# ext-sakamoro/ALICE-Codec

Hardware: AMD Instinct MI355X
Metric: Mpixels/s encode+decode, 1080p x 64 CDF9/7 q=80; bit-exact vs CPU (higher is better)
Workload: dtype int32

## Files before the change

alice-codec_amd/csrc/rans.hip:

```cpp
#include <cstdlib>

#include "common.h"
#include "freq_table.h"
#include "kernels.h"

namespace alice {


__device__ inline RansEncEntry make_enc_entry(uint32_t f, uint32_t c) {
    RansEncEntry e;
    e.freq = f;
    e.cum = c;
    unsigned long long xm = (unsigned long long)f << 19;
    unsigned long long xm8 = (unsigned long long)f << 27;
    e.xmax = xm > 0xFFFFFFFFull ? 0xFFFFFFFFu : (uint32_t)xm;
    e.xmax8 = xm8 > 0xFFFFFFFFull ? 0xFFFFFFFFu : (uint32_t)xm8;
    if (f == 0u || f > kProbScale) {
        e.xmax = f == 0u ? 0xFFFFFFFFu : e.xmax;
        e.xmax8 = f == 0u ? 0xFFFFFFFFu : e.xmax8;
        e.rcp = 0u; e.rsh = 0u; e.g = 0; e.cbias = 0u;
    } else if (f == 1u) {
        e.rcp = 0xFFFFFFFFu; e.rsh = 0u; e.g = 4095; e.cbias = c + 4095u;
    } else {
        uint32_t L = 32u - (uint32_t)__clz((int)(f - 1u));
        unsigned long long p = 1ull << (31u + L);
        e.rcp = (uint32_t)((p + f - 1u) / f);
        e.rsh = L - 1u;
        e.g = (int32_t)kProbScale - (int32_t)f;
        e.cbias = c;
    }
    return e;
}

__device__ inline uint32_t build_dec_slots(uint32_t f, uint32_t c, uint32_t* scratch, RansDecSlots* __restrict__ out) {
    const int s = threadIdx.x;
    uint32_t end = c + f;
    if (end > kProbScale) end = kProbScale;
    __syncthreads();
    scratch[s] = c;
    scratch[256 + s] = c < end ? end : c;
    scratch[512 + s] = f;
    out->symtab[s] = (f & 0xFFFFu) | (c << 16);
    __syncthreads();
    uint32_t fl = 0u;
    for (uint32_t slot = (uint32_t)s; slot < kProbScale; slot += 256u) {
        uint32_t owner = 0u;
        for (uint32_t k = 0; k < 256u; ++k)
            if (slot >= scratch[k] && slot < scratch[256 + k]) owner = k;
        const uint32_t fo = scratch[512 + owner], co = scratch[owner];
        uint32_t fe, be;
        if (fo >= kProbScale) {
            fe = 0xFFFFFFFFu; be = (slot - co) - slot + 1u;
            fl |= fo > kProbScale ? kTableDecExact : kTableDecBig;
        } else {
            fe = fo << 20; be = (slot - co) - ((fo * slot) >> kProbBits);
        }
        out->ftab[slot] = fe;
        out->btab[slot] = be;
        out->c2s[slot] = (uint8_t)owner;
    }
    return fl;
}

__global__ __launch_bounds__(256) void rans_table_kernel(const uint32_t* __restrict__ hist,
                                                         RansTable* __restrict__ tables, uint32_t n_sym,
                                                         const uint32_t* __restrict__ used) {
    __shared__ uint32_t scratch[768];
    const int chain = blockIdx.x;
    const int s = threadIdx.x;
    const uint32_t count = (uint32_t)s < n_sym ? hist[(size_t)chain * 256 + s] : 0u;
    uint32_t f, c;
    freq_table_256(count, n_sym, scratch, f, c);
    tables[chain].enc[s] = make_enc_entry(f, c);
    uint32_t fl = build_dec_slots(f, c, scratch, &tables[chain].dec);
    const uint32_t occurs = used ? used[(size_t)chain * 256 + s] : count;
    if (occurs > 0u && f == 0u) fl |= kTableDiverges;
    if (occurs > 0u && f > kProbScale) fl |= kTableNeedsGeneric;
    __shared__ uint32_t flags_sh;
    if (s == 0) flags_sh = 0u;
    __syncthreads();
    if (fl) atomicOr(&flags_sh, fl);
    __syncthreads();
    if (s == 0) tables[chain].flags = flags_sh | kTableVerified;
}

__global__ __launch_bounds__(256) void rans_table_from_arrays_kernel(const uint16_t* __restrict__ cum,
                                                                     const uint16_t* __restrict__ freq,
                                                                     RansTable* __restrict__ table) {
    __shared__ uint32_t scratch[768];
    __shared__ uint32_t flags_sh;
    const int s = threadIdx.x;
    if (s == 0) flags_sh = 0u;
    table->enc[s] = make_enc_entry(freq[s], cum[s]);
    const uint32_t fl = build_dec_slots(freq[s], cum[s], scratch, &table->dec);
    if (fl) atomicOr(&flags_sh, fl);
    __syncthreads();
    if (s == 0) table->flags = flags_sh;
}

__device__ __forceinline__ void chain_take_turns(uint32_t enabled) {
    if (!enabled) return;
    const uint32_t turn = (uint32_t)(clock64() >> 17);
    const uint32_t slot = __builtin_amdgcn_s_getreg((3 << 11) | (0 << 6) | 4);
    if ((turn ^ slot) & 1u) __builtin_amdgcn_s_setprio(1);
    else __builtin_amdgcn_s_setprio(0);
}


constexpr int kEncTile = 1024;
constexpr int kEncTilePad = 128;

__device__ __forceinline__ void ripple64(uint32_t& xin, uint32_t& xout, uint32_t xmax, uint32_t xmax8,
                                         uint32_t rcp, uint32_t rsh, int32_t g, uint32_t cprev) {
    uint32_t k, y, q;
    unsigned long long m1;
#define ALICE_RIPPLE_STEP(TAIL)                                                     \
    "v_add_u32_dpp %[xin], %[xout], %[cprev] wave_shr:1 row_mask:0xf bank_mask:0xf\n\t" \
    "v_cmp_ge_u32_e64 %[m1], %[xin], %[xmax]\n\t"                                  \
    "v_cmp_ge_u32_e32 vcc, %[xin], %[xmax8]\n\t"                                   \
    "s_nop 0\n\t"                                                                    \
    "v_cndmask_b32_e64 %[k], 0, 8, %[m1]\n\t"                                      \
    "v_cndmask_b32_e64 %[k], %[k], 16, vcc\n\t"                                    \
    "v_lshrrev_b32_e32 %[y], %[k], %[xin]\n\t"                                     \
    "v_mul_hi_u32 %[q], %[y], %[rcp]\n\t"                                          \
    "v_lshrrev_b32_e32 %[q], %[rsh], %[q]\n\t"                                     \
    "v_mad_i32_i24 %[xout], %[q], %[g], %[y]\n\t" TAIL
#define ALICE_RIPPLE_STEP4 ALICE_RIPPLE_STEP("s_nop 1\n\t") ALICE_RIPPLE_STEP("s_nop 1\n\t") ALICE_RIPPLE_STEP("s_nop 1\n\t") ALICE_RIPPLE_STEP("s_nop 1\n\t")
#define ALICE_RIPPLE_STEP16 ALICE_RIPPLE_STEP4 ALICE_RIPPLE_STEP4 ALICE_RIPPLE_STEP4 ALICE_RIPPLE_STEP4
    asm volatile(
        "s_nop 1\n\t"
        ALICE_RIPPLE_STEP16 ALICE_RIPPLE_STEP16 ALICE_RIPPLE_STEP16 ALICE_RIPPLE_STEP16
        : [xin] "+v"(xin), [xout] "+v"(xout), [k] "=&v"(k), [y] "=&v"(y), [q] "=&v"(q), [m1] "=&s"(m1)
        : [xmax] "v"(xmax), [xmax8] "v"(xmax8), [rcp] "v"(rcp), [rsh] "v"(rsh), [g] "v"(g),
          [cprev] "v"(cprev)
        : "vcc");
#undef ALICE_RIPPLE_STEP16
#undef ALICE_RIPPLE_STEP4
#undef ALICE_RIPPLE_STEP
}

__device__ __forceinline__ void ripple64_clean(uint32_t& xin, uint32_t& xout, uint32_t thr, uint32_t k0, uint32_t k1,
                                               uint32_t rcp, uint32_t rsh, int32_t g, uint32_t cprev) {
    uint32_t k, y, q;
#define ALICE_RIPPLE_STEP                                                            \
    "v_add_u32_dpp %[xin], %[xout], %[cprev] wave_shr:1 row_mask:0xf bank_mask:0xf\n\t" \
    "v_cmp_ge_u32_e32 vcc, %[xin], %[thr]\n\t"                                     \
    "s_nop 1\n\t"                                                                  \
    "v_cndmask_b32_e32 %[k], %[k0], %[k1], vcc\n\t"                                \
    "v_lshrrev_b32_e32 %[y], %[k], %[xin]\n\t"                                     \
    "v_mul_hi_u32 %[q], %[y], %[rcp]\n\t"                                          \
    "v_lshrrev_b32_e32 %[q], %[rsh], %[q]\n\t"                                     \
    "v_mad_i32_i24 %[xout], %[q], %[g], %[y]\n\t"                                  \
    "s_nop 1\n\t"
#define ALICE_RIPPLE_STEP4 ALICE_RIPPLE_STEP ALICE_RIPPLE_STEP ALICE_RIPPLE_STEP ALICE_RIPPLE_STEP
#define ALICE_RIPPLE_STEP16 ALICE_RIPPLE_STEP4 ALICE_RIPPLE_STEP4 ALICE_RIPPLE_STEP4 ALICE_RIPPLE_STEP4
    asm volatile(
        "s_nop 1\n\t"
        ALICE_RIPPLE_STEP16 ALICE_RIPPLE_STEP16 ALICE_RIPPLE_STEP16 ALICE_RIPPLE_STEP16
        : [xin] "+v"(xin), [xout] "+v"(xout), [k] "=&v"(k), [y] "=&v"(y), [q] "=&v"(q)
        : [thr] "v"(thr), [k0] "v"(k0), [k1] "v"(k1), [rcp] "v"(rcp), [rsh] "v"(rsh), [g] "v"(g), [cprev] "v"(cprev)
        : "vcc");
#undef ALICE_RIPPLE_STEP16
#undef ALICE_RIPPLE_STEP4
#undef ALICE_RIPPLE_STEP
}

__device__ __forceinline__ void ripple64_comp(uint32_t& u, uint32_t& z, uint32_t kc, uint32_t tpp, uint32_t rcp, uint32_t rsh,
                                              int32_t g) {
    uint32_t m, q;
#define ALICE_RIPPLE_STEP                                                            \
    "v_add_u32_dpp %[u], %[z], %[kc] wave_shr:1 row_mask:0xf bank_mask:0xf\n\t"     \
    "v_mad_i64_i32 v[62:63], vcc, %[u], %[two24], v[60:61]\n\t"                    \
    "v_min_u32_e32 %[m], %[u], v63\n\t"                                           \
    "v_mul_hi_u32 %[q], %[m], %[rcp]\n\t"                                          \
    "v_lshrrev_b32_e32 %[q], %[rsh], %[q]\n\t"                                     \
    "v_mad_i32_i24 %[z], %[q], %[g], %[m]\n\t"                                     \
    "s_nop 1\n\t"
#define ALICE_RIPPLE_STEP4 ALICE_RIPPLE_STEP ALICE_RIPPLE_STEP ALICE_RIPPLE_STEP ALICE_RIPPLE_STEP
#define ALICE_RIPPLE_STEP16 ALICE_RIPPLE_STEP4 ALICE_RIPPLE_STEP4 ALICE_RIPPLE_STEP4 ALICE_RIPPLE_STEP4
    asm volatile(
        "v_mov_b32_e32 v60, 0\n\t"
        "v_mov_b32_e32 v61, %[tpp]\n\t"
        ALICE_RIPPLE_STEP16 ALICE_RIPPLE_STEP16 ALICE_RIPPLE_STEP16 ALICE_RIPPLE_STEP16
        : [u] "+v"(u), [z] "=&v"(z), [m] "=&v"(m), [q] "=&v"(q)
        : [kc] "v"(kc), [tpp] "v"(tpp), [rcp] "v"(rcp), [rsh] "v"(rsh), [g] "v"(g), [two24] "s"(1u << 24)
        : "v60", "v61", "v62", "v63", "vcc");
#undef ALICE_RIPPLE_STEP16
#undef ALICE_RIPPLE_STEP4
#undef ALICE_RIPPLE_STEP
}

template <bool kExclusive>
__global__ __launch_bounds__(64) void rans_encode_kernel(const uint8_t* __restrict__ sym_base,
                                                         unsigned long long sym_stride,
                                                         unsigned long long n_first,
                                                         const RansTable* __restrict__ tables,
                                                         uint8_t* __restrict__ out_base,
                                                         unsigned long long cap0,
                                                         unsigned long long group_stride,
                                                         unsigned long long group_head,
                                                         unsigned n_split,
                                                         RansResult* __restrict__ results,
                                                         unsigned long long cap1, unsigned long long cap2,
                                                         uint32_t x_init, uint32_t keep_open, uint32_t take_turns,
                                                         const RansEncodeDesc* __restrict__ descs) {
    __shared__ uint4 tab_a[256];
    __shared__ uint4 tab_b[256];
    __shared__ uint2 tab_c[256];
    __shared__ __attribute__((aligned(16))) uint8_t tile[kEncTilePad + kEncTile];

    if constexpr (kExclusive) asm volatile("" ::: "a255");
    const int chain = blockIdx.x;
    const int lane = threadIdx.x;
    unsigned long long n = n_first - (((unsigned)chain >= n_split && n_first > 0ull) ? 1ull : 0ull);
    const uint8_t* __restrict__ sym = sym_base + (size_t)chain * sym_stride;
    const RansTable* __restrict__ tbl = tables + chain;
    const int gch = chain % 3;
    unsigned long long cap = group_stride == 0ull ? cap0 : (gch == 0 ? cap0 : (gch == 1 ? cap1 : cap2));
    uint8_t* region = group_stride == 0ull ? out_base + (size_t)chain * cap0
                                           : out_base + (size_t)(chain / 3) * group_stride + group_head +
                                                 (gch == 0 ? 0ull : (gch == 1 ? cap0 : cap0 + cap1));
    RansResult* res = results + chain;
    if (descs) {
        const RansEncodeDesc ds = descs[chain];
        sym = ds.sym; n = ds.n; tbl = ds.table; region = ds.region; cap = ds.cap; res = ds.result;
        x_init = ds.x_init; keep_open = ds.keep_open;
    }
    uint8_t* const out_end = region + cap;
    uint8_t* const dummy = region + lane;

    for (int s = lane; s < 256; s += 64) {
        const RansEncEntry e = tbl->enc[s];
        tab_a[s] = make_uint4(e.xmax, e.rcp, e.rsh, (uint32_t)e.g);
        tab_b[s] = make_uint4(e.xmax - (e.xmax >> 8), e.cbias + e.freq + ((1u << 31) - kProbScale - 1u), e.cbias, e.xmax8);
        tab_c[s] = make_uint2(e.freq, e.cum);
    }

    const uint32_t tbl_flags = (uint32_t)__builtin_amdgcn_readfirstlane((int)tbl->flags);
    const bool table_clean = x_init == kRansL && (tbl_flags & (kTableVerified | kTableNeedsGeneric | kTableDiverges)) == kTableVerified;
    uint32_t x = x_init;
    const unsigned long long clk0 = clock64(), rt0 = wall_clock64();
    unsigned long long written = 0ull;
    uint32_t flags = 0u;
    uint32_t paths = 0u, load_paths = 0u, slow_tiles = 0u, comp_blocks = 0u;
    asm volatile("" : "+v"(load_paths));

    const unsigned long long ntiles = (n + kEncTile - 1) / kEncTile;
    auto load_tile = [&](unsigned long long j) -> uint4 {
        uint4 v = make_uint4(0u, 0u, 0u, 0u);
        if (j >= ntiles) return v;
        const long long hi = (long long)(n - j * kEncTile);
        const long long lo = hi - kEncTile + 16ll * lane;
        if (lo >= 0) {
            const uint8_t* p = sym + lo;
            const uint32_t mis = (uint32_t)((uintptr_t)p & 3u);
            const uint32_t* p4 = (const uint32_t*)(p - mis);
            if (mis == 0u) {
                v = make_uint4(p4[0], p4[1], p4[2], p4[3]);
            } else if (lo + 20 <= (long long)n || mis == 0u) {
                const uint32_t t0 = p4[0], t1 = p4[1], t2 = p4[2], t3 = p4[3], t4 = p4[4];
                const uint32_t sh = mis * 8u;
                load_paths |= kEncPathFunnel;
                v = make_uint4((t0 >> sh) | (t1 << (32u - sh)), (t1 >> sh) | (t2 << (32u - sh)),
                               (t2 >> sh) | (t3 << (32u - sh)), (t3 >> sh) | (t4 << (32u - sh)));
            } else {
                uint32_t w[4] = {0u, 0u, 0u, 0u};
                for (int b = 0; b < 16; ++b) w[b >> 2] |= (uint32_t)p[b] << (8 * (b & 3));
                v = make_uint4(w[0], w[1], w[2], w[3]);
                load_paths |= kEncPathBytewiseEnd;
            }
        } else {
            uint32_t w[4] = {0u, 0u, 0u, 0u};
            for (int b = 0; b < 16; ++b) {
                const long long idx = lo + b;
                if (idx >= 0) w[b >> 2] |= (uint32_t)sym[idx] << (8 * (b & 3));
            }
            v = make_uint4(w[0], w[1], w[2], w[3]);
            load_paths |= kEncPathBytewiseHead;
        }
        return v;
    };

    struct BlockParams { uint4 ea, eb; uint2 ec; };
    auto sym_of = [&](int b) -> uint32_t { return tile[kEncTilePad + kEncTile - 1 - lane - b * 64]; };
    auto params_of = [&](uint32_t s) -> BlockParams { BlockParams p; p.ea = tab_a[s]; p.eb = tab_b[s]; p.ec = tab_c[s]; return p; };

    uint4 cur = load_tile(0);
    for (unsigned long long j = 0; j < ntiles; ++j) {
        if (!kExclusive && (j & 7ull) == 0ull) chain_take_turns(take_turns);
        __syncthreads();
        ((uint4*)(tile + kEncTilePad))[lane] = cur;
        __syncthreads();
        cur = load_tile(j + 1);
        const long long hi = (long long)(n - j * kEncTile);
        const int valid = hi >= kEncTile ? kEncTile : (int)hi;
        const int nblocks = (valid + 63) / 64;

        uint32_t sym1 = sym_of(1);
        BlockParams nxt = params_of(sym_of(0));
        if (table_clean && valid == kEncTile && written + 2ull * kEncTile + 4ull + 320ull <= cap) {
            uint32_t xin = x;
            constexpr uint32_t kTileSpan = 2u * kEncTile + 320u;
            const uintptr_t tb_v = (uintptr_t)(out_end - written - kTileSpan);
            typedef __attribute__((address_space(1))) uint8_t GlobalByte;
            GlobalByte* const tb = (GlobalByte*)(((uintptr_t)(uint32_t)__builtin_amdgcn_readfirstlane((int)(uint32_t)(tb_v >> 32)) << 32) |
                                                 (uintptr_t)(uint32_t)__builtin_amdgcn_readfirstlane((int)(uint32_t)tb_v));
            uint32_t tw = 0u, rare_blocks = 0u;
            asm volatile("" : "+v"(tw));
#pragma unroll 2
            for (int b = 0; b < kEncTile / 64; ++b) {
                const BlockParams curp = nxt;
                nxt = params_of(sym1);
                sym1 = sym_of(b + 2);
                const uint32_t xmax = curp.ea.x, rcp = curp.ea.y, rsh = curp.ea.z;
                const int32_t g = (int32_t)curp.ea.w;
                const bool small_f = xmax <= kRansL;
                if (__builtin_expect(__ballot(small_f) == 0ull, 1)) {
                    const uint32_t tm1 = xmax - 1u, tpp = curp.eb.x, cc = curp.eb.y;
                    uint32_t cc_prev = (uint32_t)__builtin_amdgcn_update_dpp(0, (int)cc, 0x138, 0xf, 0xf, true);
                    asm volatile("" : "+v"(cc_prev));
                    const uint32_t kc = tm1 - cc_prev;
                    uint32_t u = tm1 - xin, z;
                    ripple64_comp(u, z, kc, tpp, rcp, rsh, g);
                    const bool c1 = (int32_t)u < 0;
                    const unsigned long long b1 = __ballot(c1);
                    const uint32_t off = __builtin_amdgcn_mbcnt_hi((uint32_t)(b1 >> 32), __builtin_amdgcn_mbcnt_lo((uint32_t)b1, tw));
                    tb[c1 ? kTileSpan - 1u - off : (uint32_t)lane] = (uint8_t)(~u & 0xFFu);
                    tw += (uint32_t)__popcll(b1);
                    xin = (uint32_t)__builtin_amdgcn_update_dpp(0, (int)(cc - z), 0x13C, 0xf, 0xf, true);
                } else {
                    rare_blocks += 1u;
                    const uint32_t cbias = curp.eb.z, xmax8 = curp.eb.w;
                    uint32_t xout = 0u;
                    const uint32_t cprev = (uint32_t)__builtin_amdgcn_update_dpp(0, (int)cbias, 0x138, 0xf, 0xf, true);
                    const uint32_t k0 = small_f ? 8u : 0u;
                    ripple64_clean(xin, xout, small_f ? xmax8 : xmax, k0, k0 + 8u, rcp, rsh, g, cprev);
                    const bool c1 = xin >= xmax;
                    const bool c2 = xin >= xmax8;
                    const unsigned long long b1 = __ballot(c1), b2 = __ballot(c2);
                    const uint32_t off = __builtin_amdgcn_mbcnt_hi((uint32_t)(b1 >> 32), __builtin_amdgcn_mbcnt_lo((uint32_t)b1, tw)) +
                                         __builtin_amdgcn_mbcnt_hi((uint32_t)(b2 >> 32), __builtin_amdgcn_mbcnt_lo((uint32_t)b2, 0u));
                    tb[c1 ? kTileSpan - 1u - off : (uint32_t)lane] = (uint8_t)(xin & 0xFFu);
                    tb[c2 ? kTileSpan - 2u - off : (uint32_t)lane] = (uint8_t)((xin >> 8) & 0xFFu);
                    tw += (uint32_t)__popcll(b1) + (uint32_t)__popcll(b2);
                    xin = (uint32_t)__builtin_amdgcn_update_dpp(0, (int)(xout + cbias), 0x13C, 0xf, 0xf, false);
                }
                asm volatile("" : "+v"(tw));
            }
            written += (unsigned long long)(uint32_t)__builtin_amdgcn_readfirstlane((int)tw);
            comp_blocks += (uint32_t)(kEncTile / 64) - rare_blocks;
            x = (uint32_t)__builtin_amdgcn_readlane((int)xin, 0);
            continue;
        }
        slow_tiles += 1u;
        paths |= valid < kEncTile ? kEncPathTail : (table_clean ? kEncPathCapRefused : kEncPathNotClean);
        for (int b = 0; b < nblocks; ++b) {
            const BlockParams curp = nxt;
            nxt = params_of(sym1);
            sym1 = sym_of(b + 2);
            const bool active = (kEncTile - 1 - (b * 64 + lane)) >= kEncTile - valid;
            uint4 ea = curp.ea;
            uint4 eb = curp.eb;
            uint2 ec = curp.ec;
            if (!active) {
                ea = make_uint4(0xFFFFFFFFu, 0u, 0u, 0u);
                eb = make_uint4(0u, 0u, 0u, 0xFFFFFFFFu);
                ec = make_uint2(1u, 0u);
            }
            const uint32_t xmax = ea.x, xmax8 = eb.w, rcp = ea.y, rsh = ea.z;
            const int32_t g = (int32_t)ea.w;
            const uint32_t cbias = eb.z, freq = ec.x, cum = ec.y;
            const bool bad = (freq - 1u) >= kProbScale;

            uint32_t xin = x, xout = 0u;
            if (__builtin_expect(__ballot(bad) == 0ull, 1)) {
                uint32_t cprev = (uint32_t)__builtin_amdgcn_update_dpp(0, (int)cbias, 0x138, 0xf, 0xf, true);
                ripple64(xin, xout, xmax, xmax8, rcp, rsh, g, cprev);
                x = (uint32_t)__builtin_amdgcn_readlane((int)xout, 63) +
                    (uint32_t)__builtin_amdgcn_readlane((int)cbias, 63);
            } else {
                paths |= kEncPathExact;
                uint32_t xs = x;
                for (int i = 0; i < 64; ++i) {
                    if (lane == i) xin = xs;
                    const uint32_t fi = (uint32_t)__builtin_amdgcn_readlane((int)freq, i);
                    const uint32_t ci = (uint32_t)__builtin_amdgcn_readlane((int)cum, i);
                    const uint32_t ai = (uint32_t)__builtin_amdgcn_readlane((int)active, i);
                    if (!ai) continue;
                    if (fi == 0u) { flags |= kTableDiverges; continue; }
                    const unsigned long long xm = (unsigned long long)fi << 19;
                    uint32_t ys = xs;
                    while ((unsigned long long)ys >= xm) ys >>= 8;
                    const uint32_t qs = ys / fi, rs = ys % fi;
                    xs = (qs << kProbBits) + rs + ci;
                }
                x = xs;
            }

            const bool c1 = xin >= xmax;
            const bool c2 = xin >= xmax8;
            const unsigned long long b1 = __ballot(c1), b2 = __ballot(c2);
            const uint32_t off = __builtin_amdgcn_mbcnt_hi((uint32_t)(b1 >> 32), __builtin_amdgcn_mbcnt_lo((uint32_t)b1, 0u)) +
                                 __builtin_amdgcn_mbcnt_hi((uint32_t)(b2 >> 32), __builtin_amdgcn_mbcnt_lo((uint32_t)b2, 0u));
            const uint32_t total = (uint32_t)__popcll(b1) + (uint32_t)__popcll(b2);
            const bool room = written + total + 4ull + 64ull <= cap;
            flags |= room ? 0u : kRansOverflow;
            paths |= room ? 0u : kEncPathNoRoom;
            uint8_t* p = out_end - 1 - (written + off);
            uint8_t* p0 = (c1 && room) ? p : dummy;
            uint8_t* p1 = (c2 && room) ? p - 1 : dummy;
            *p0 = (uint8_t)(xin & 0xFFu);
            *p1 = (uint8_t)((xin >> 8) & 0xFFu);
            written += total;
        }
    }

    if (!keep_open) {
        if (written + 4ull + 64ull <= cap) {
            if (lane < 4) out_end[-1 - (long long)(written + lane)] = (uint8_t)((x >> (8 * lane)) & 0xFFu);
        } else {
            flags |= kRansOverflow;
            paths |= kEncPathNoRoom;
        }
        written += 4ull;
    }
    for (uint32_t bit = kEncPathFunnel; bit <= kEncPathBytewiseHead; bit <<= 1)
        paths |= __ballot((load_paths & bit) != 0u) ? bit : 0u;
    const uint32_t clean_tiles = (uint32_t)ntiles - slow_tiles;
    paths |= clean_tiles ? kEncPathClean : 0u;
    if (lane == 0) {
        res->len = written;
        res->flags = flags;
        res->final_state = x;
        res->fast_tiles = clean_tiles;
        res->slow_tiles = slow_tiles;
        res->paths = paths;
        res->comp_blocks = comp_blocks;
        res->cycles_k = (uint32_t)((clock64() - clk0) >> 10);
        res->ticks_k = (uint32_t)((wall_clock64() - rt0) >> 10);
        res->hw_id = __builtin_amdgcn_s_getreg((31 << 11) | 4);
        res->xcc_id = __builtin_amdgcn_s_getreg((31 << 11) | 20);
    }
}


constexpr int kDecBlocks = 64;
constexpr int kDecTile = kDecBlocks * 64;
constexpr int kDecWinBytes = 33 * 64 * 4;
constexpr int kDecWinLds = kDecWinBytes;

#include "rans_decode_tile.inc"

__device__ __forceinline__ void dec_tile_fast(uint32_t& x, uint32_t& pos, const RansDecSlots* slots, uint32_t lane4,
                                              uint32_t win_addr, uint32_t rec_addr, uint32_t nblk) {
    uint32_t xo, po;
    asm volatile(ALICE_DEC_TILE_ASM
                 : [xo] "=&s"(xo), [po] "=&s"(po), [ra] "+v"(rec_addr)
                 : [xi] "s"(x), [pi] "s"(pos), [nb] "s"(nblk), [tp] "s"(slots), [l4] "v"(lane4), [wa] "v"(win_addr)
                 : ALICE_DEC_TILE_CLOBBERS);
    x = xo;
    pos = po;
}

__device__ __forceinline__ void dec_tile_dry(uint32_t& x, const RansDecSlots* slots, uint32_t lane4, uint32_t rec_addr, uint32_t nblk) {
    uint32_t xo;
    asm volatile(ALICE_DEC_DRY_TILE_ASM
                 : [xo] "=&s"(xo), [ra] "+v"(rec_addr)
                 : [xi] "s"(x), [nb] "s"(nblk), [tp] "s"(slots), [l4] "v"(lane4)
                 : ALICE_DEC_DRY_TILE_CLOBBERS);
    x = xo;
}

template <bool kExclusive>
__global__ __launch_bounds__(64) void rans_decode_kernel(const RansDecodeDesc* __restrict__ descs,
                                                         RansResult* __restrict__ results, uint32_t take_turns) {
    if constexpr (kExclusive) asm volatile("" ::: "a63");
    __shared__ __attribute__((aligned(16))) uint8_t c2s[kProbScale];
    __shared__ uint32_t symtab[256];
    __shared__ __attribute__((aligned(16))) uint8_t win[kDecWinLds];
    __shared__ __attribute__((aligned(16))) uint16_t rec[kDecTile];
    uint8_t* const obuf = (uint8_t*)rec;

    const RansDecodeDesc d = descs[blockIdx.x];
    const int lane = threadIdx.x;
    const RansDecSlots* const slots = &d.table->dec;
    uint32_t flags = 0u;
    const uint32_t tflags = d.table->flags;
    const bool big_freq = (tflags & kTableDecBig) != 0u;
    const bool exact_only = (tflags & kTableDecExact) != 0u;
    for (int i = lane; i < (int)kProbScale / 16; i += 64) ((uint4*)c2s)[i] = ((const uint4*)slots->c2s)[i];
    for (int i = lane; i < 256; i += 64) symtab[i] = slots->symtab[i];
    __syncthreads();
    bool slot0_big = false, one_owner = false;
    if (big_freq) {
        const uint32_t o0 = c2s[0];
        slot0_big = symtab[o0] == kProbScale;
        bool same = true;
        for (int i = lane; i < (int)kProbScale; i += 64) same &= c2s[i] == o0;
        one_owner = __ballot(!same) == 0ull;
    }

    uint32_t x = 0u;
    unsigned long long pos = 0ull;
    const unsigned long long len = d.in_len;
    if (d.resume) {
        x = d.x0; pos = d.pos0;
    } else if (len >= 4ull) {
        x = ((uint32_t)d.in[0] << 24) | ((uint32_t)d.in[1] << 16) | ((uint32_t)d.in[2] << 8) | (uint32_t)d.in[3];
        pos = 4ull;
    }
    bool pending = false;
    const unsigned long long clk0 = clock64(), rt0 = wall_clock64();
    unsigned long long done = 0ull;
    uint32_t n_fast = 0u, n_slow = 0u, paths = 0u;

    while (done < d.n) {
        if (!kExclusive) chain_take_turns(take_turns);
        const unsigned long long remain = d.n - done;
        const uint32_t want = remain < (unsigned long long)kDecTile ? (uint32_t)remain : (uint32_t)kDecTile;
        const bool dry_ok = !exact_only && (!slot0_big || (one_owner && x != 0u));
        if (want == (uint32_t)kDecTile && pos >= len && dry_ok) {
            uint32_t xs = (uint32_t)__builtin_amdgcn_readfirstlane((int)x);
            __syncthreads();
            dec_tile_dry(xs, slots, 4u * lane, (uint32_t)(uintptr_t)rec + 2u * lane, (uint32_t)kDecBlocks);
            x = xs;
            __syncthreads();
            const bool out_al = (((uintptr_t)(d.out + done)) & 3u) == 0u;
            paths |= kDecPathDry | (out_al ? 0u : kDecPathUnaligned);
            for (int i = lane * 4; i < kDecTile; i += 256) {
                const uint2 r4 = *(const uint2*)&rec[i];
                const uint32_t packed = (uint32_t)c2s[r4.x & (kProbScale - 1u)] | ((uint32_t)c2s[(r4.x >> 16) & (kProbScale - 1u)] << 8) |
                                        ((uint32_t)c2s[r4.y & (kProbScale - 1u)] << 16) | ((uint32_t)c2s[(r4.y >> 16) & (kProbScale - 1u)] << 24);
                if (out_al) *(uint32_t*)(d.out + done + i) = packed;
                else for (int b = 0; b < 4; ++b) d.out[done + i + b] = (uint8_t)(packed >> (8 * b));
            }
            done += (unsigned long long)kDecTile;
            ++n_fast;
            continue;
        }
        unsigned long long wbase = pos & ~3ull;
        {
            const unsigned long long mis = (unsigned long long)((uintptr_t)(d.in + pos) & 3u);
            if (pos >= mis) wbase = pos - mis;
        }
        const bool whole = (len - wbase >= (unsigned long long)kDecWinLds) && ((((uintptr_t)(d.in + wbase)) & 3u) == 0u);
        __syncthreads();
        if (whole) {
            const uint32_t* g = (const uint32_t*)(d.in + wbase) + lane;
            uint32_t wv[kDecWinLds / 256];
#pragma unroll
            for (int k = 0; k < kDecWinLds / 256; ++k) wv[k] = g[k * 64];
#pragma unroll
            for (int k = 0; k < kDecWinLds / 256; ++k) ((uint32_t*)win)[k * 64 + lane] = wv[k];
        } else {
            for (int i = lane * 4; i < kDecWinLds; i += 64 * 4) {
                const unsigned long long o = wbase + (unsigned long long)i;
                uint32_t w = 0u;
                for (int b = 0; b < 4; ++b)
                    if (o + (unsigned long long)b < len) w |= (uint32_t)d.in[o + b] << (8 * b);
                *(uint32_t*)(win + i) = w;
            }
        }
        __syncthreads();

        uint32_t got = 0u;
        bool fast = (want == (uint32_t)kDecTile) && pos < len && !exact_only;
        const uint32_t x_save = x;
        const unsigned long long pos_save = pos;
        const bool pending_save = pending;
        if (fast && pending) {
            uint32_t xs = x;
            unsigned long long ps = pos;
            int guard = 0;
            while (xs < kRansL && ps < len && guard < 8) { xs = (xs << 8) | (uint32_t)win[ps - wbase]; ps += 1ull; ++guard; }
            if (xs < kRansL) { fast = false; paths |= kDecPathStillStarved; }
            else { x = xs; pos = ps; pending = false; paths |= kDecPathPendingFed; }
        }
        if (fast && x < kRansL) { fast = false; paths |= kDecPathBelowL; }
        if (fast) {
            uint32_t prel = (uint32_t)(pos - wbase);
            uint32_t xs = (uint32_t)__builtin_amdgcn_readfirstlane((int)x);
            prel = (uint32_t)__builtin_amdgcn_readfirstlane((int)prel);
            dec_tile_fast(xs, prel, slots, 4u * lane, (uint32_t)(uintptr_t)win + 4u * lane,
                          (uint32_t)(uintptr_t)rec + 2u * lane, (uint32_t)kDecBlocks);
            x = xs;
            pos = wbase + prel;
            pending = false;
            __syncthreads();
            if (pos > len) {
                x = x_save; pos = pos_save; pending = pending_save;
                fast = false;
                paths |= kDecPathSpecDropped;
            } else {
                paths |= whole ? kDecPathWhole : kDecPathSpecKept;
            }
        }
        if (fast) {
            const bool out_aligned = (((uintptr_t)(d.out + done)) & 3u) == 0u;
            for (int i = lane * 4; i < kDecTile; i += 256) {
                const uint2 r4 = *(const uint2*)&rec[i];
                const uint32_t packed = (uint32_t)c2s[r4.x & (kProbScale - 1u)] | ((uint32_t)c2s[(r4.x >> 16) & (kProbScale - 1u)] << 8) |
                                        ((uint32_t)c2s[r4.y & (kProbScale - 1u)] << 16) | ((uint32_t)c2s[(r4.y >> 16) & (kProbScale - 1u)] << 24);
                if (out_aligned) *(uint32_t*)(d.out + done + i) = packed;
                else *(uint32_t*)(obuf + i) = packed;
            }
            paths |= out_aligned ? 0u : kDecPathUnaligned;
            got = out_aligned ? 0u : (uint32_t)kDecTile;
            done += out_aligned ? (unsigned long long)kDecTile : 0ull;
            ++n_fast;
        } else {
            ++n_slow;
            paths |= kDecPathExact | (want < (uint32_t)kDecTile ? kDecPathTail : 0u);
            __shared__ uint32_t sh_state, sh_cnt, sh_starved;
            __shared__ unsigned long long sh_pos;
            if (lane == 0) {
                uint32_t j = 0u, xs = x;
                unsigned long long ps = pos;
                bool pend = pending;
                const unsigned long long wend = wbase + (unsigned long long)kDecWinBytes;
                bool starved = false;
                while (j < want) {
                    if (pend) {
                        while (xs < kRansL && ps < len) {
                            if (ps >= wend) { starved = true; break; }
                            xs = (xs << 8) | (uint32_t)win[ps - wbase];
                            ps += 1ull;
                        }
                        if (starved) break;
                    }
                    const uint32_t slot = xs & (kProbScale - 1u);
                    const uint32_t sy = c2s[slot];
                    const uint32_t fc = symtab[sy];
                    xs = (fc & 0xFFFFu) * (xs >> kProbBits) + slot - (fc >> 16);
                    obuf[j] = (uint8_t)sy;
                    pend = true;
                    ++j;
                }
                sh_state = xs; sh_pos = ps; sh_cnt = j; sh_starved = starved ? 1u : 0u;
            }
            __syncthreads();
            x = sh_state; pos = sh_pos; got = sh_cnt;
            paths |= sh_starved ? kDecPathStarved : 0u;
            pending = true;
        }
        __syncthreads();
        for (uint32_t i = lane; i < got; i += 64) d.out[done + i] = obuf[i];
        done += got;
    }
    if (pending) {
        while (x < kRansL && pos < len) { x = (x << 8) | (uint32_t)d.in[pos]; pos += 1ull; }
    }
    if (lane == 0) {
        RansResult* const res = d.result ? d.result : results + blockIdx.x;
        res->len = pos;
        res->flags = flags;
        res->final_state = x;
        res->fast_tiles = n_fast;
        res->slow_tiles = n_slow;
        res->paths = paths;
        res->cycles_k = (uint32_t)((clock64() - clk0) >> 10);
        res->ticks_k = (uint32_t)((wall_clock64() - rt0) >> 10);
        res->hw_id = __builtin_amdgcn_s_getreg((31 << 11) | 4);
        res->xcc_id = __builtin_amdgcn_s_getreg((31 << 11) | 20);
    }
}


void launch_rans_table(const uint32_t* d_hist, RansTable* d_tables, int n_chains, hipStream_t st, uint32_t n_symbols,
                       const uint32_t* d_used) {
    if (n_chains <= 0) return;
    hipLaunchKernelGGL(rans_table_kernel, dim3(n_chains), dim3(256), 0, st, d_hist, d_tables, n_symbols, d_used);
}

void launch_rans_table_from_arrays(const uint16_t* d_cum, const uint16_t* d_freq, RansTable* d_table,
                                   hipStream_t st) {
    hipLaunchKernelGGL(rans_table_from_arrays_kernel, dim3(1), dim3(256), 0, st, d_cum, d_freq, d_table);
}

static uint32_t chain_turns_enabled() {
    static const uint32_t on = [] { const char* v = getenv("ALICE_CHAIN_TURNS"); return (v && *v == '1') ? 1u : 0u; }();
    return on;
}

static unsigned chain_lds_pad(int n_chains, unsigned static_lds) {
    if (n_chains <= 1024 || n_chains > 2048) return 0u;
    const unsigned want = 163840u / 8u - 1024u;
    return want > static_lds ? want - static_lds : 0u;
}

struct ChainKernelFacts { bool ok; unsigned enc_regs, enc_lds, enc_wg_per_cu, dec_regs, dec_lds, dec_wg_per_cu, enc_lds_plain, dec_lds_plain; };
static const ChainKernelFacts& chain_kernel_facts() {
    static const ChainKernelFacts f = [] {
        ChainKernelFacts r{};
        hipFuncAttributes a{};
        int nb = 0;
        r.ok = true;
        auto q = [&](const void* fn, unsigned& regs, unsigned& lds, unsigned* wg) {
            if (hipFuncGetAttributes(&a, fn) != hipSuccess) { r.ok = false; (void)hipGetLastError(); return; }
            regs = (unsigned)a.numRegs; lds = (unsigned)a.sharedSizeBytes;
            if (wg) {
                if (hipOccupancyMaxActiveBlocksPerMultiprocessor(&nb, fn, 64, 0) != hipSuccess) { r.ok = false; (void)hipGetLastError(); return; }
                *wg = (unsigned)nb;
            }
        };
        unsigned dummy = 0;
        q((const void*)rans_encode_kernel<true>, r.enc_regs, r.enc_lds, &r.enc_wg_per_cu);
        q((const void*)rans_decode_kernel<true>, r.dec_regs, r.dec_lds, &r.dec_wg_per_cu);
        q((const void*)rans_encode_kernel<false>, dummy, r.enc_lds_plain, nullptr);
        q((const void*)rans_decode_kernel<false>, dummy, r.dec_lds_plain, nullptr);
        return r;
    }();
    return f;
}
bool chain_kernel_occupancy(uint32_t out[6]) {
    const ChainKernelFacts& f = chain_kernel_facts();
    out[0] = f.enc_regs; out[1] = f.enc_lds; out[2] = f.enc_wg_per_cu;
    out[3] = f.dec_regs; out[4] = f.dec_lds; out[5] = f.dec_wg_per_cu;
    return f.ok;
}

void launch_rans_encode(const uint8_t* d_sym, uint64_t sym_stride, uint64_t n, const RansTable* d_tables,
                        uint8_t* d_out, uint64_t cap, RansResult* d_results, int n_chains, hipStream_t st,
                        uint64_t group_stride, uint64_t group_head, unsigned n_split, uint64_t cap_co, uint64_t cap_cg,
                        uint32_t x_init, bool keep_open) {
    if (n_chains <= 0) return;
    auto kern = n_chains <= 1024 ? rans_encode_kernel<true> : rans_encode_kernel<false>;
    const ChainKernelFacts& facts = chain_kernel_facts();
    hipLaunchKernelGGL(kern, dim3(n_chains), dim3(64), chain_lds_pad(n_chains, facts.ok ? facts.enc_lds_plain : 9216u), st, d_sym,
                       (unsigned long long)sym_stride, (unsigned long long)n, d_tables, d_out,
                       (unsigned long long)cap, (unsigned long long)group_stride, (unsigned long long)group_head, n_split,
                       d_results, (unsigned long long)(cap_co ? cap_co : cap), (unsigned long long)(cap_cg ? cap_cg : cap),
                       x_init, keep_open ? 1u : 0u, chain_turns_enabled(), (const RansEncodeDesc*)nullptr);
}

void launch_rans_encode_descs(const RansEncodeDesc* d_descs, int n_chains, hipStream_t st) {
    if (n_chains <= 0) return;
    auto kern = n_chains <= 1024 ? rans_encode_kernel<true> : rans_encode_kernel<false>;
    const ChainKernelFacts& facts = chain_kernel_facts();
    hipLaunchKernelGGL(kern, dim3(n_chains), dim3(64), chain_lds_pad(n_chains, facts.ok ? facts.enc_lds_plain : 9216u), st,
                       (const uint8_t*)nullptr, 0ull, 0ull, (const RansTable*)nullptr, (uint8_t*)nullptr, 0ull, 0ull, 0ull, 0xFFFFFFFFu,
                       (RansResult*)nullptr, 0ull, 0ull, kRansL, 0u, chain_turns_enabled(), d_descs);
}

void launch_rans_decode(const RansDecodeDesc* d_descs, RansResult* d_results, int n_chains, hipStream_t st) {
    if (n_chains <= 0) return;
    auto kern = n_chains <= 1024 ? rans_decode_kernel<true> : rans_decode_kernel<false>;
    const ChainKernelFacts& facts = chain_kernel_facts();
    hipLaunchKernelGGL(kern, dim3(n_chains), dim3(64), chain_lds_pad(n_chains, facts.ok ? facts.dec_lds_plain : 21776u + 256u), st, d_descs, d_results,
                       chain_turns_enabled());
}

}
```

Baseline: 11820.

## Fuse consecutive rANS encode blocks into one software-pipelined inline-asm run

Replaces the per-block ripple64_comp call with a looping inline-asm routine that processes consecutive compressible blocks back-to-back. Each iteration hides the next block's LDS table and symbol reads, parameter setup and the previous block's byte store and ballot bookkeeping inside the s_nop slots of the serial DPP ripple chain. Register sets alternate between blocks. The two enc tables are merged into one contiguous LDS array so a single base address plus offset serves both reads. This adds heavy hand scheduling with hardcoded VGPRs, which risks hazards and subtle correctness problems.

```diff
diff --git a/alice-codec_amd/csrc/rans.hip b/alice-codec_amd/csrc/rans.hip
--- a/alice-codec_amd/csrc/rans.hip
+++ b/alice-codec_amd/csrc/rans.hip
@@ -165,29 +165,94 @@
 #undef ALICE_RIPPLE_STEP
 }
 
-__device__ __forceinline__ void ripple64_comp(uint32_t& u, uint32_t& z, uint32_t kc, uint32_t tpp, uint32_t rcp, uint32_t rsh,
-                                              int32_t g) {
-    uint32_t m, q;
-#define ALICE_RIPPLE_STEP                                                            \
-    "v_add_u32_dpp %[u], %[z], %[kc] wave_shr:1 row_mask:0xf bank_mask:0xf\n\t"     \
-    "v_mad_i64_i32 v[62:63], vcc, %[u], %[two24], v[60:61]\n\t"                    \
-    "v_min_u32_e32 %[m], %[u], v63\n\t"                                           \
-    "v_mul_hi_u32 %[q], %[m], %[rcp]\n\t"                                          \
-    "v_lshrrev_b32_e32 %[q], %[rsh], %[q]\n\t"                                     \
-    "v_mad_i32_i24 %[z], %[q], %[g], %[m]\n\t"                                     \
-    "s_nop 1\n\t"
-#define ALICE_RIPPLE_STEP4 ALICE_RIPPLE_STEP ALICE_RIPPLE_STEP ALICE_RIPPLE_STEP ALICE_RIPPLE_STEP
-#define ALICE_RIPPLE_STEP16 ALICE_RIPPLE_STEP4 ALICE_RIPPLE_STEP4 ALICE_RIPPLE_STEP4 ALICE_RIPPLE_STEP4
+
+struct CompSet { uint32_t kc, rcp, rsh, cc; int32_t g; };
+struct CompNext { uint32_t xmax, tpp, cbias, xmax8, tm1; };
+
+__device__ __forceinline__ void ripple64_comp_run(uint32_t& u0, uint32_t& u1, uint32_t& z, uint32_t tpp, CompSet& sa_, CompSet& sb_,
+                                                  uint32_t tab, uint32_t& ad, uint32_t& sa, uint32_t& sym1, CompNext& nx,
+                                                  unsigned long long& stop, uint32_t& left, uint32_t& phase, uint32_t& tw,
+                                                  uint32_t lane, uint32_t span1, const void* tb) {
+    uint32_t m, q, ccp, cnt, off, byt;
+    unsigned long long cy, end, tp = (unsigned long long)tpp << 32;
+#define ALICE_RUN_CHAIN(CTRL, U, S)                                                          \
+    "v_add_u32_dpp %[" U "], %[z], %[kc" S "] " CTRL " row_mask:0xf bank_mask:0xf\n\t"      \
+    "v_mad_i64_i32 v[62:63], %[cy], %[" U "], %[two24], %[tp]\n\t"                          \
+    "v_min_u32_e32 %[m], %[" U "], v63\n\t"                                                 \
+    "v_mul_hi_u32 %[q], %[m], %[rcp" S "]\n\t"                                              \
+    "v_lshrrev_b32_e32 %[q], %[rsh" S "], %[q]\n\t"                                         \
+    "v_mad_i32_i24 %[z], %[q], %[g" S "], %[m]\n\t"
+#define ALICE_RUN_STEP(U, S, FILL) ALICE_RUN_CHAIN("wave_shr:1", U, S) FILL
+#define ALICE_RUN_IDLE(U, S) ALICE_RUN_STEP(U, S, "s_nop 1\n\t")
+#define ALICE_RUN_IDLE4(U, S) ALICE_RUN_IDLE(U, S) ALICE_RUN_IDLE(U, S) ALICE_RUN_IDLE(U, S) ALICE_RUN_IDLE(U, S)
+#define ALICE_RUN_IDLE13(U, S) ALICE_RUN_IDLE4(U, S) ALICE_RUN_IDLE4(U, S) ALICE_RUN_IDLE4(U, S) ALICE_RUN_IDLE(U, S)
+#define ALICE_RUN_REST(U, S, N)                                                                                                   \
+    ALICE_RUN_IDLE13(U, S)                                                                                                        \
+    ALICE_RUN_STEP(U, S, "s_waitcnt lgkmcnt(0)\n\t s_nop 1\n\t")                                                                 \
+    ALICE_RUN_STEP(U, S, "v_lshl_add_u32 %[ad], %[sy], 4, %[tab]\n\t v_cmp_ge_u32_e64 %[sm], %[rl], v52\n\t")                    \
+    ALICE_RUN_STEP(U, S, "v_mov_b32_dpp %[ccp], %[cc" S "] wave_ror:1 row_mask:0xf bank_mask:0xf\n\t s_nop 0\n\t")              \
+    ALICE_RUN_STEP(U, S, "v_mov_b32_dpp %[ccp], v57 wave_shr:1 row_mask:0xf bank_mask:0xf\n\t s_nop 0\n\t")                      \
+    ALICE_RUN_STEP(U, S, "v_add_u32_e32 %[tmn], -1, v52\n\t s_nop 0\n\t")                                                        \
+    ALICE_RUN_STEP(U, S, "v_sub_u32_e32 %[kc" N "], %[tmn], %[ccp]\n\t s_nop 0\n\t")                                             \
+    ALICE_RUN_STEP(U, S, "v_mov_b32_e32 %[rcp" N "], v53\n\t v_mov_b32_e32 %[rsh" N "], v54\n\t")                                \
+    ALICE_RUN_STEP(U, S, "v_mov_b32_e32 %[g" N "], v55\n\t v_mov_b32_e32 %[cc" N "], v57\n\t")                                   \
+    ALICE_RUN_STEP(U, S, "v_mov_b32_e32 %[xmn], v52\n\t v_mov_b32_e32 %[cbn], v58\n\t")                                          \
+    ALICE_RUN_STEP(U, S, "v_mov_b32_e32 %[x8n], v59\n\t v_mov_b32_e32 %[tpn], v56\n\t")                                          \
+    ALICE_RUN_STEP(U, S, "s_cmp_eq_u32 %[left], 0\n\t s_cselect_b64 %[end], -1, 0\n\t")                                          \
+    ALICE_RUN_STEP(U, S, "s_or_b64 %[sm], %[sm], %[end]\n\t s_sub_u32 %[left], %[left], 1\n\t")                                  \
+    ALICE_RUN_IDLE13(U, S) ALICE_RUN_IDLE13(U, S) ALICE_RUN_IDLE4(U, S) ALICE_RUN_IDLE(U, S)                                      \
+    ALICE_RUN_STEP(U, S, "v_lshlrev_b64 %[tp], 32, v[56:57]\n\t s_cmp_lg_u64 %[sm], 0\n\t")
+#define ALICE_RUN_READ_A "ds_read_b128 v[52:55], %[ad]\n\t"
+#define ALICE_RUN_READ_B "ds_read_b128 v[56:59], %[ad] offset:4096\n\t"
+#define ALICE_RUN_READ_S "ds_read_u8 %[sy], %[sa]\n\t"
+#define ALICE_RUN_FIRST(U, S, N)                                                                                                  \
+    ALICE_RUN_STEP(U, S, ALICE_RUN_READ_A " s_nop 0\n\t")                                                                         \
+    ALICE_RUN_IDLE(U, S)                                                                                                          \
+    ALICE_RUN_STEP(U, S, ALICE_RUN_READ_B " s_nop 0\n\t")                                                                         \
+    ALICE_RUN_STEP(U, S, ALICE_RUN_READ_S " s_nop 0\n\t")                                                                         \
+    ALICE_RUN_IDLE(U, S) ALICE_RUN_IDLE(U, S)                                                                                     \
+    ALICE_RUN_STEP(U, S, "v_subrev_u32_e32 %[sa], 64, %[sa]\n\t s_nop 0\n\t")                                                    \
+    ALICE_RUN_REST(U, S, N)
+#define ALICE_RUN_NEXT(U, P, S, N)                                                                                                \
+    ALICE_RUN_CHAIN("wave_ror:1", U, S) "v_cmp_gt_i32_e32 vcc, 0, %[" P "]\n\t" ALICE_RUN_READ_A                                  \
+    ALICE_RUN_STEP(U, S, "v_not_b32_e32 %[byt], %[" P "]\n\t s_bcnt1_i32_b64 %[cnt], vcc\n\t")                                   \
+    ALICE_RUN_STEP(U, S, "v_mbcnt_lo_u32_b32 %[off], vcc_lo, %[tw]\n\t" ALICE_RUN_READ_B)                                         \
+    ALICE_RUN_STEP(U, S, "v_mbcnt_hi_u32_b32 %[off], vcc_hi, %[off]\n\t" ALICE_RUN_READ_S)                                        \
+    ALICE_RUN_STEP(U, S, "v_sub_u32_e32 %[off], %[span1], %[off]\n\t v_add_u32_e32 %[tw], %[cnt], %[tw]\n\t")                    \
+    ALICE_RUN_STEP(U, S, "v_cndmask_b32_e32 %[off], %[lane], %[off], vcc\n\t s_nop 0\n\t")                                       \
+    ALICE_RUN_STEP(U, S, "global_store_byte %[off], %[byt], %[tb]\n\t v_subrev_u32_e32 %[sa], 64, %[sa]\n\t")                    \
+    ALICE_RUN_REST(U, S, N)
     asm volatile(
-        "v_mov_b32_e32 v60, 0\n\t"
-        "v_mov_b32_e32 v61, %[tpp]\n\t"
-        ALICE_RIPPLE_STEP16 ALICE_RIPPLE_STEP16 ALICE_RIPPLE_STEP16 ALICE_RIPPLE_STEP16
-        : [u] "+v"(u), [z] "=&v"(z), [m] "=&v"(m), [q] "=&v"(q)
-        : [kc] "v"(kc), [tpp] "v"(tpp), [rcp] "v"(rcp), [rsh] "v"(rsh), [g] "v"(g), [two24] "s"(1u << 24)
-        : "v60", "v61", "v62", "v63", "vcc");
-#undef ALICE_RIPPLE_STEP16
-#undef ALICE_RIPPLE_STEP4
-#undef ALICE_RIPPLE_STEP
+        "s_mov_b32 %[ph], 0\n\t"
+        ALICE_RUN_FIRST("u0", "a", "b")
+        "1:\n\t"
+        "s_cbranch_scc1 3f\n\t"
+        ALICE_RUN_NEXT("u1", "u0", "b", "a")
+        "s_cbranch_scc1 2f\n\t"
+        ALICE_RUN_NEXT("u0", "u1", "a", "b")
+        "s_branch 1b\n\t"
+        "2:\n\t"
+        "s_mov_b32 %[ph], 1\n\t"
+        "3:\n\t"
+        : [u0] "+v"(u0), [u1] "=&v"(u1), [z] "=&v"(z), [tp] "+v"(tp), [ad] "+v"(ad), [sa] "+v"(sa), [sy] "=&v"(sym1), [tw] "+v"(tw),
+          [off] "=&v"(off), [byt] "=&v"(byt), [cnt] "=&s"(cnt), [m] "=&v"(m), [q] "=&v"(q), [ccp] "=&v"(ccp), [cy] "=&s"(cy),
+          [sm] "=&s"(stop), [end] "=&s"(end), [left] "+s"(left), [ph] "=&s"(phase), [tmn] "=&v"(nx.tm1), [xmn] "=&v"(nx.xmax),
+          [tpn] "=&v"(nx.tpp), [cbn] "=&v"(nx.cbias), [x8n] "=&v"(nx.xmax8),
+          [kca] "+v"(sa_.kc), [rcpa] "+v"(sa_.rcp), [rsha] "+v"(sa_.rsh), [ga] "+v"(sa_.g), [cca] "+v"(sa_.cc),
+          [kcb] "=&v"(sb_.kc), [rcpb] "=&v"(sb_.rcp), [rshb] "=&v"(sb_.rsh), [gb] "=&v"(sb_.g), [ccb] "=&v"(sb_.cc)
+        : [tab] "s"(tab), [lane] "v"(lane), [span1] "s"(span1), [two24] "s"(1u << 24), [rl] "s"(kRansL), [tb] "s"(tb)
+        : "v52", "v53", "v54", "v55", "v56", "v57", "v58", "v59", "v62", "v63", "vcc", "scc", "memory");
+#undef ALICE_RUN_NEXT
+#undef ALICE_RUN_FIRST
+#undef ALICE_RUN_READ_S
+#undef ALICE_RUN_READ_B
+#undef ALICE_RUN_READ_A
+#undef ALICE_RUN_REST
+#undef ALICE_RUN_IDLE13
+#undef ALICE_RUN_IDLE4
+#undef ALICE_RUN_IDLE
+#undef ALICE_RUN_STEP
+#undef ALICE_RUN_CHAIN
 }
 
 template <bool kExclusive>
@@ -204,8 +269,7 @@
                                                          unsigned long long cap1, unsigned long long cap2,
                                                          uint32_t x_init, uint32_t keep_open, uint32_t take_turns,
                                                          const RansEncodeDesc* __restrict__ descs) {
-    __shared__ uint4 tab_a[256];
-    __shared__ uint4 tab_b[256];
+    __shared__ uint4 tab_ab[512];
     __shared__ uint2 tab_c[256];
     __shared__ __attribute__((aligned(16))) uint8_t tile[kEncTilePad + kEncTile];
 
@@ -231,8 +295,8 @@
 
     for (int s = lane; s < 256; s += 64) {
         const RansEncEntry e = tbl->enc[s];
-        tab_a[s] = make_uint4(e.xmax, e.rcp, e.rsh, (uint32_t)e.g);
-        tab_b[s] = make_uint4(e.xmax - (e.xmax >> 8), e.cbias + e.freq + ((1u << 31) - kProbScale - 1u), e.cbias, e.xmax8);
+        tab_ab[s] = make_uint4(e.xmax, e.rcp, e.rsh, (uint32_t)e.g);
+        tab_ab[256 + s] = make_uint4(e.xmax - (e.xmax >> 8), e.cbias + e.freq + ((1u << 31) - kProbScale - 1u), e.cbias, e.xmax8);
         tab_c[s] = make_uint2(e.freq, e.cum);
     }
 
@@ -283,7 +347,7 @@
 
     struct BlockParams { uint4 ea, eb; uint2 ec; };
     auto sym_of = [&](int b) -> uint32_t { return tile[kEncTilePad + kEncTile - 1 - lane - b * 64]; };
-    auto params_of = [&](uint32_t s) -> BlockParams { BlockParams p; p.ea = tab_a[s]; p.eb = tab_b[s]; p.ec = tab_c[s]; return p; };
+    auto params_of = [&](uint32_t s) -> BlockParams { BlockParams p; p.ea = tab_ab[s]; p.eb = tab_ab[256 + s]; p.ec = tab_c[s]; return p; };
 
     uint4 cur = load_tile(0);
     for (unsigned long long j = 0; j < ntiles; ++j) {
@@ -307,34 +371,48 @@
                                                  (uintptr_t)(uint32_t)__builtin_amdgcn_readfirstlane((int)(uint32_t)tb_v));
             uint32_t tw = 0u, rare_blocks = 0u;
             asm volatile("" : "+v"(tw));
-#pragma unroll 2
-            for (int b = 0; b < kEncTile / 64; ++b) {
-                const BlockParams curp = nxt;
-                nxt = params_of(sym1);
-                sym1 = sym_of(b + 2);
-                const uint32_t xmax = curp.ea.x, rcp = curp.ea.y, rsh = curp.ea.z;
-                const int32_t g = (int32_t)curp.ea.w;
-                const bool small_f = xmax <= kRansL;
-                if (__builtin_expect(__ballot(small_f) == 0ull, 1)) {
-                    const uint32_t tm1 = xmax - 1u, tpp = curp.eb.x, cc = curp.eb.y;
-                    uint32_t cc_prev = (uint32_t)__builtin_amdgcn_update_dpp(0, (int)cc, 0x138, 0xf, 0xf, true);
-                    asm volatile("" : "+v"(cc_prev));
-                    const uint32_t kc = tm1 - cc_prev;
-                    uint32_t u = tm1 - xin, z;
-                    ripple64_comp(u, z, kc, tpp, rcp, rsh, g);
+            uint32_t xmax = nxt.ea.x, tpp = nxt.eb.x, cbias = nxt.eb.z, xmax8 = nxt.eb.w;
+            CompSet cs;
+            cs.rcp = nxt.ea.y; cs.rsh = nxt.ea.z; cs.g = (int32_t)nxt.ea.w; cs.cc = nxt.eb.y;
+            const uint32_t tab = (uint32_t)(uintptr_t)tab_ab;
+            uint32_t ad = tab + 16u * sym1;
+            uint32_t sa = (uint32_t)(uintptr_t)tile + (uint32_t)(kEncTilePad + kEncTile - 1 - 2 * 64) - (uint32_t)lane;
+            auto kc_of = [](uint32_t tm1_, uint32_t cc_) -> uint32_t {
+                uint32_t cc_prev = (uint32_t)__builtin_amdgcn_update_dpp(0, (int)cc_, 0x138, 0xf, 0xf, true);
+                asm volatile("" : "+v"(cc_prev));
+                return tm1_ - cc_prev;
+            };
+            unsigned long long stop = __ballot(xmax <= kRansL);
+            uint32_t tm1 = xmax - 1u;
+            cs.kc = kc_of(tm1, cs.cc);
+            uint32_t left = (uint32_t)(kEncTile / 64 - 1);
+            while ((int32_t)left >= 0) {
+                if (__builtin_expect(stop == 0ull, 1)) {
+                    CompSet sa_ = cs, sb_;
+                    CompNext nx;
+                    uint32_t u0 = tm1 - xin, u1, z, phase;
+                    ripple64_comp_run(u0, u1, z, tpp, sa_, sb_, tab, ad, sa, sym1, nx, stop, left, phase, tw, (uint32_t)lane,
+                                      kTileSpan - 1u, (const void*)tb);
+                    const bool swapped = phase != 0u;
+                    const uint32_t u = swapped ? u1 : u0, cc_last = swapped ? sb_.cc : sa_.cc;
+                    cs.kc = swapped ? sa_.kc : sb_.kc; cs.rcp = swapped ? sa_.rcp : sb_.rcp; cs.rsh = swapped ? sa_.rsh : sb_.rsh;
+                    cs.g = swapped ? sa_.g : sb_.g; cs.cc = swapped ? sa_.cc : sb_.cc;
+                    xmax = nx.xmax; tpp = nx.tpp; cbias = nx.cbias; xmax8 = nx.xmax8; tm1 = nx.tm1;
                     const bool c1 = (int32_t)u < 0;
                     const unsigned long long b1 = __ballot(c1);
-                    const uint32_t off = __builtin_amdgcn_mbcnt_hi((uint32_t)(b1 >> 32), __builtin_amdgcn_mbcnt_lo((uint32_t)b1, tw));
-                    tb[c1 ? kTileSpan - 1u - off : (uint32_t)lane] = (uint8_t)(~u & 0xFFu);
+                    const uint32_t o1 = __builtin_amdgcn_mbcnt_hi((uint32_t)(b1 >> 32), __builtin_amdgcn_mbcnt_lo((uint32_t)b1, tw));
+                    tb[c1 ? kTileSpan - 1u - o1 : (uint32_t)lane] = (uint8_t)(~u & 0xFFu);
                     tw += (uint32_t)__popcll(b1);
-                    xin = (uint32_t)__builtin_amdgcn_update_dpp(0, (int)(cc - z), 0x13C, 0xf, 0xf, true);
+                    xin = (uint32_t)__builtin_amdgcn_update_dpp(0, (int)(cc_last - z), 0x13C, 0xf, 0xf, true);
                 } else {
                     rare_blocks += 1u;
-                    const uint32_t cbias = curp.eb.z, xmax8 = curp.eb.w;
+                    const BlockParams np = params_of(sym1);
+                    sym1 = sym_of(kEncTile / 64 + 1 - (int)left);
+                    const bool small_f = xmax <= kRansL;
                     uint32_t xout = 0u;
                     const uint32_t cprev = (uint32_t)__builtin_amdgcn_update_dpp(0, (int)cbias, 0x138, 0xf, 0xf, true);
                     const uint32_t k0 = small_f ? 8u : 0u;
-                    ripple64_clean(xin, xout, small_f ? xmax8 : xmax, k0, k0 + 8u, rcp, rsh, g, cprev);
+                    ripple64_clean(xin, xout, small_f ? xmax8 : xmax, k0, k0 + 8u, cs.rcp, cs.rsh, cs.g, cprev);
                     const bool c1 = xin >= xmax;
                     const bool c2 = xin >= xmax8;
                     const unsigned long long b1 = __ballot(c1), b2 = __ballot(c2);
@@ -344,6 +422,12 @@
                     tb[c2 ? kTileSpan - 2u - off : (uint32_t)lane] = (uint8_t)((xin >> 8) & 0xFFu);
                     tw += (uint32_t)__popcll(b1) + (uint32_t)__popcll(b2);
                     xin = (uint32_t)__builtin_amdgcn_update_dpp(0, (int)(xout + cbias), 0x13C, 0xf, 0xf, false);
+                    xmax = np.ea.x; cs.rcp = np.ea.y; cs.rsh = np.ea.z; cs.g = (int32_t)np.ea.w;
+                    tpp = np.eb.x; cs.cc = np.eb.y; cbias = np.eb.z; xmax8 = np.eb.w;
+                    stop = __ballot(xmax <= kRansL);
+                    tm1 = xmax - 1u; cs.kc = kc_of(tm1, cs.cc);
+                    ad = tab + 16u * sym1; sa -= 64u;
+                    left -= 1u;
                 }
                 asm volatile("" : "+v"(tw));
             }
```

Result: faster. 11940, median of 6 (+1.1%).
